# churchill-lab/alntools

Hardware: AMD Instinct MI355X
Metric: alignments/sec BAM->EC (100M PE reads, 8-hap) at 1/2/4/8 MI355X (higher is better)
Workload: dtype u32

## Files before the change

alntools_amd/csrc/ecb.hip:

```cpp
#include <hip/hip_runtime.h>

#include <algorithm>
#include <climits>
#include <cstddef>
#include <cstdarg>
#include <cstdio>
#include <cstring>
#include <cstdlib>
#include <memory>
#include <mutex>
#include <string>
#include <vector>

#include "../../include/ecb.h"

namespace {

typedef unsigned long long u64;
typedef unsigned int u32;
typedef unsigned short u16;

constexpr int TPB = 256;
constexpr u32 MAX_PROBE = 256;
constexpr u32 PENDING = 0xFFFFFFFFu;
constexpr u32 ARENA_CHUNK = 512;
constexpr u32 QSTRIPES = 64;
constexpr u32 ARENA_REGIONS = 64;
constexpr u32 MAX_LOCI = (1u << 26) - 2u;
constexpr u32 MAX_LOCI_SHORT = (1u << 25) - 2u;
constexpr u32 INL = 5;
constexpr u32 DEAD_KEY = 0xFFFFFFFFu;
constexpr u32 SPIN_MAX = 1u << 16;

constexpr u32 ERR_CONTRACT = 1u;
// ... 1549 lines not shown
    const int* ptr = cscptr + (u64)h * (n_loci + 1);
    const u64 j = g - hap_start[h];
    u32 lo = 0, hi = n_loci;
    while (lo < hi) { const u32 m = (lo + hi + 1) >> 1; if ((u64)ptr[m] <= j) lo = m; else hi = m - 1; }
    keys[g] = (u64)(u32)cscidx[g] * n_loci + lo;
    vals[g] = 1u << h;
}
__global__ void k_cv_back_emit(const u64* keys, const u32* vals, const u32* flag, const u32* pos, u64 total, u32 n_loci,
                               int* indices, int* data) {
    const u64 i = blockIdx.x * (u64)blockDim.x + threadIdx.x;
    if (i >= total || !flag[i]) return;
    u32 m = 0;
    for (u64 j = i; j < total && keys[j] == keys[i]; ++j) m |= vals[j];
    indices[pos[i]] = (int)(keys[i] % n_loci);
    data[pos[i]] = (int)m;
}
__global__ void k_cv_back_rowptr(const u64* keys, const u32* pos, u64 total, u32 nnz, u32 n_ecs, u32 n_loci, int* indptr) {
    const u64 e = blockIdx.x * (u64)blockDim.x + threadIdx.x;
    if (e > n_ecs) return;
    const u64 at = lower_bound_u64(keys, total, (u64)e * n_loci);
    indptr[e] = at < total ? (int)pos[at] : (int)nnz;
}

constexpr int CVB = 1024;
__global__ __launch_bounds__(TPB) void k_cv_bits(const int* data, u64 nnz, u64* total) {
    u64 v = 0;
    for (u64 i = blockIdx.x * (u64)TPB + threadIdx.x; i < nnz; i += (u64)gridDim.x * TPB) v += __popc((u32)data[i]);
#pragma unroll
    for (int d = 32; d > 0; d >>= 1) v += __shfl_xor(v, d);
    if ((threadIdx.x & 63u) == 0 && v) atomicAdd(total, v);
}
__global__ void k_cv_keys(const int* indptr, u32 n_ecs, const int* indices, const int* data, u64 nnz, u32 n_loci, u32 n_haps,
                          u64* keys, u32* vals, u32* err) {
    const u64 e = blockIdx.x * (u64)blockDim.x + threadIdx.x;
    if (e >= n_ecs) return;
    const long long a = indptr[e], b = indptr[e + 1];
    if (a < 0 || b < a || (u64)b > nnz || (e == 0 && a != 0)) { atomicOr(err, 1u); return; }
    bool bad = false;
    for (long long i = a; i < b; ++i) {
        const u32 lc = (u32)indices[i], m = (u32)data[i];
        bad |= lc >= n_loci || m == 0u || (m >> n_haps) != 0u;
        keys[i] = ((u64)lc << 32) | (u32)e;
        vals[i] = m;
    }
    if (bad) atomicOr(err, 2u);
}
__global__ __launch_bounds__(TPB) void k_cv_cnt(const u32* masks, u64 nnz, u32 n_haps, u32 nb, u32* blk) {
    __shared__ u32 cnt[32];
    if (threadIdx.x < 32) cnt[threadIdx.x] = 0;
    __syncthreads();
    const u64 i0 = (u64)blockIdx.x * CVB;
#pragma unroll
    for (int r = 0; r < CVB / TPB; ++r) {
        const u64 i = i0 + (u64)r * TPB + threadIdx.x;
        const u32 m = i < nnz ? masks[i] : 0u;
        for (u32 h = 0; h < n_haps; ++h) {
            const u64 bm = __ballot((m >> h) & 1u);
            if ((threadIdx.x & 63u) == 0 && bm) atomicAdd(&cnt[h], (u32)__popcll(bm));
        }
    }
    __syncthreads();
    if (threadIdx.x < n_haps) blk[(u64)threadIdx.x * nb + blockIdx.x] = cnt[threadIdx.x];
}
template <bool VAL>
__global__ __launch_bounds__(TPB) void k_cv_emit(const u64* keys, const u32* masks, u64 nnz, u32 n_haps, u32 n_loci, u32 nb,
                                                 const u32* scan, int* cscidx, u32* headval, const u32* base, const double* values,
                                                 double* cscdata) {
    __shared__ u32 run[32], wcnt[TPB / 64][32];
    const u32 tid = threadIdx.x, lane = tid & 63u, w = tid >> 6;
    if (tid < 32) run[tid] = tid < n_haps ? scan[(u64)tid * nb + blockIdx.x] : 0u;
    const u64 lt = (1ull << lane) - 1ull;
    const u64 i0 = (u64)blockIdx.x * CVB;
    for (int r = 0; r < CVB / TPB; ++r) {
        const u64 i = i0 + (u64)r * TPB + tid;
        const bool have = i < nnz;
        const u64 key = have ? keys[i] : 0ull;
        const u32 m = have ? masks[i] : 0u;
        const u32 lc = (u32)(key >> 32);
        const bool head = have && (i == 0 || (u32)(keys[i - 1] >> 32) != lc);
        for (u32 h = 0; h < n_haps; ++h) {
            const u64 bm = __ballot((m >> h) & 1u);
            if (lane == 0) wcnt[w][h] = (u32)__popcll(bm);
        }
        __syncthreads();
        for (u32 h = 0; h < n_haps; ++h) {
            const u64 bm = __ballot((m >> h) & 1u);
            u32 at = run[h] + (u32)__popcll(bm & lt);
            for (u32 k = 0; k < w; ++k) at += wcnt[k][h];
            if ((m >> h) & 1u) {
                cscidx[at] = (int)(u32)key;
                if (VAL) cscdata[at] = values[base[i] + (u32)__popc(m & ((1u << h) - 1u))];
            }
            if (head) headval[(u64)h * n_loci + lc] = at - scan[(u64)h * nb];
        }
        __syncthreads();
        if (tid < n_haps) { u32 c = 0; for (u32 k = 0; k < TPB / 64; ++k) c += wcnt[k][tid]; run[tid] += c; }
        __syncthreads();
    }
}
__global__ void k_cv_ptr(const u64* keys, u64 nnz, u32 n_loci, u32 n_haps, u32 nb, const u32* scan, const u64* grand, const u32* headval, int* cscptr) {
    const u64 t = blockIdx.x * (u64)blockDim.x + threadIdx.x;
    if (t > n_loci) return;
    const u64 at = lower_bound_u64(keys, nnz, t << 32);
    const u32 t2 = at < nnz ? (u32)(keys[at] >> 32) : 0u;
    for (u32 h = 0; h < n_haps; ++h) {
        const u32 tot = (h + 1 < n_haps ? scan[(u64)(h + 1) * nb] : (u32)*grand) - scan[(u64)h * nb];
        cscptr[(u64)h * (n_loci + 1) + t] = (int)(at < nnz ? headval[(u64)h * n_loci + t2] : tot);
    }
}

__global__ __launch_bounds__(TPB) void k_cvv_bits(const int* data, u64 nnz, u32* bits) {
    const u64 i = blockIdx.x * (u64)TPB + threadIdx.x;
    if (i < nnz) bits[i] = (u32)__popc((u32)data[i]);
}
__global__ __launch_bounds__(TPB) void k_cvv_gather(const u32* idx, const int* data, const u32* bits_excl, u64 nnz, u32* masks, u32* base) {
    const u64 p = blockIdx.x * (u64)TPB + threadIdx.x;
    if (p >= nnz) return;
    const u32 i = idx[p];
    masks[p] = (u32)data[i];
    base[p] = bits_excl[i];
}

__global__ void k_iota(u32* out, u64 n) {
    const u64 i = blockIdx.x * (u64)blockDim.x + threadIdx.x;
    if (i < n) out[i] = (u32)i;
}
__global__ void k_read_ec(const u32* read_slot, u64 n, const u32* rank_of_slot, int* out) {
    const u64 i = blockIdx.x * (u64)blockDim.x + threadIdx.x;
    if (i < n) out[i] = read_slot[i] == 0xFFFFFFFFu ? -1 : (int)rank_of_slot[read_slot[i]];
// ... 15 lines not shown
    const u64 s = A.start[blockIdx.y], n = A.len[blockIdx.y];
    for (u64 i = blockIdx.x * (u64)blockDim.x + threadIdx.x; i < n; i += (u64)gridDim.x * blockDim.x) arena[s + i] = make_uint2(0u, 0u);
}
__global__ void k_clear_slots(Slot* table, const u32* list, u64 n) {
    const u64 i = blockIdx.x * (u64)blockDim.x + threadIdx.x;
    if (i >= n) return;
    uint4* s = reinterpret_cast<uint4*>(table + list[i]);
    const uint4 z = make_uint4(0, 0, 0, 0);
    s[0] = z; s[1] = z; s[2] = z; s[3] = z;
}

#ifndef ECB_RS_TPB
#define ECB_RS_TPB 1024
#endif
constexpr int RS_TPB = ECB_RS_TPB, RS_TILE = 4096, RS_ITEMS = RS_TILE / RS_TPB;
static_assert(RS_TPB >= 256 && RS_TPB % 64 == 0 && RS_TILE % RS_TPB == 0, "one thread per digit among the first 256");
constexpr int RS_MAX_PASSES = 8;
constexpr u32 RS_AGG = 1u << 30, RS_PFX = 2u << 30, RS_VAL = (1u << 30) - 1u;
constexpr u32 RS_SPIN_MAX = 1u << 24;
#ifndef ECB_RS_LOOK
#define ECB_RS_LOOK 4
#endif
constexpr int RS_LOOK = ECB_RS_LOOK;
struct RsShifts { u32 s[RS_MAX_PASSES]; u32 n; };
__global__ __launch_bounds__(RS_TPB) void k_rs_hist_all(const u64* keys, u64 n, RsShifts sh, u32* ghist) {
    __shared__ u32 h[RS_MAX_PASSES][256];
    for (u32 q = threadIdx.x; q < RS_MAX_PASSES * 256; q += RS_TPB) (&h[0][0])[q] = 0;
    __syncthreads();
    for (u64 i = blockIdx.x * (u64)RS_TPB + threadIdx.x; i < n; i += (u64)gridDim.x * RS_TPB) {
        const u64 k = keys[i];
        for (u32 p = 0; p < sh.n; ++p) atomicAdd(&h[p][(u32)(k >> sh.s[p]) & 255u], 1u);
    }
    __syncthreads();
    if (threadIdx.x < 256u) for (u32 p = 0; p < sh.n; ++p) { const u32 c = h[p][threadIdx.x]; if (c) atomicAdd(&ghist[p * 256 + threadIdx.x], c); }
}
__global__ __launch_bounds__(256) void k_rs_bases(const u32* ghist, u32 n_passes, u32* base) {
    __shared__ u32 s_w[4];
    for (u32 p = 0; p < n_passes; ++p) {
        const u32 v = ghist[p * 256 + threadIdx.x];
        const u32 incl = wave_incl_scan(v);
        if ((threadIdx.x & 63u) == 63u) s_w[threadIdx.x >> 6] = incl;
        __syncthreads();
        u32 before = 0;
        for (u32 k = 0; k < (threadIdx.x >> 6); ++k) before += s_w[k];
        base[p * 256 + threadIdx.x] = before + incl - v;
        __syncthreads();
    }
}
__global__ __launch_bounds__(RS_TPB) void k_rs_pass(const u64* kin, const u32* vin, u64 n, u32 shift, const u32* base, u32* desc,
                                                    u32* ticket, u32* err, u64* kout, u32* vout) {
    __shared__ u32 cnt[RS_TPB / 64][256];
    __shared__ u32 dstart[256];
    __shared__ u32 gbase[256];
    __shared__ u32 s_wsum[RS_TPB / 64];
    __shared__ u32 s_tile;
    __shared__ u64 skey[RS_TILE];
    __shared__ u32 sval[RS_TILE];
    const u32 tid = threadIdx.x, lane = tid & 63u, w = tid >> 6;
    if (tid == 0) s_tile = atomicAdd(ticket, 1u);
    for (u32 q = tid; q < (RS_TPB / 64) * 256; q += RS_TPB) (&cnt[0][0])[q] = 0;
    __syncthreads();
    const u32 tile = s_tile;
    const u64 t0 = (u64)tile * RS_TILE;
    if (t0 >= n) return;
    const u64 w0 = t0 + (u64)w * (RS_TILE / (RS_TPB / 64));
    const u64 lt = (1ull << lane) - 1ull;
    u64 key[RS_ITEMS];
    u32 val[RS_ITEMS], rk[RS_ITEMS];
#pragma unroll
    for (int r = 0; r < RS_ITEMS; ++r) {
        const u64 i = w0 + (u64)r * 64 + lane;
        const bool have = i < n;
        key[r] = have ? kin[i] : 0ull;
        val[r] = have ? vin[i] : 0u;
        const u32 d = (u32)(key[r] >> shift) & 255u;
        u64 peers = __ballot(have);
#pragma unroll
        for (int b = 0; b < 8; ++b) {
            const u64 m = __ballot((d >> b) & 1u);
            peers &= ((d >> b) & 1u) ? m : ~m;
        }
        const u32 below = (u32)__popcll(peers & lt);
        u32 bs = 0;
        if (have && below == 0u) bs = atomicAdd(&cnt[w][d], (u32)__popcll(peers));
        bs = __shfl(bs, have ? __ffsll((long long)peers) - 1 : (int)lane);
        rk[r] = bs + below;
    }
    __syncthreads();
    u32 tot = 0;
    const bool dig = tid < 256u;
    const u32 dt = dig ? tid : 0u;
    if (dig) {
#pragma unroll
        for (int k = 0; k < RS_TPB / 64; ++k) { const u32 c = cnt[k][tid]; cnt[k][tid] = tot; tot += c; }
    }
    u32* const mine = desc + (u64)tile * 256 + dt;
    u32 excl = 0;
    if (!dig) {
    } else if (tile == 0) {
        __hip_atomic_store(mine, RS_PFX | tot, __ATOMIC_RELAXED, __HIP_MEMORY_SCOPE_AGENT);
    } else {
        __hip_atomic_store(mine, RS_AGG | tot, __ATOMIC_RELAXED, __HIP_MEMORY_SCOPE_AGENT);
        u32 spins = 0;
        bool done = false;
        for (long long t = (long long)tile - 1; t >= 0 && !done;) {
            u32 v[RS_LOOK];
#pragma unroll
            for (int k = 0; k < RS_LOOK; ++k)
                v[k] = t - k >= 0 ? __hip_atomic_load(desc + (u64)(t - k) * 256 + dt, __ATOMIC_RELAXED, __HIP_MEMORY_SCOPE_AGENT) : 0u;
            int used = 0;
#pragma unroll
            for (int k = 0; k < RS_LOOK; ++k) {
                if (done || used != k || t - k < 0) continue;
                if (v[k] < RS_AGG) continue;
                excl += v[k] & RS_VAL;
                used = k + 1;
                if (v[k] >= RS_PFX) done = true;
            }
            t -= used;
            if (!used) {
                if (++spins > RS_SPIN_MAX) { atomicOr(err, 1u); break; }
                __builtin_amdgcn_s_sleep(1);
            }
        }
        __hip_atomic_store(mine, RS_PFX | ((excl + tot) & RS_VAL), __ATOMIC_RELAXED, __HIP_MEMORY_SCOPE_AGENT);
    }
    if (dig) gbase[tid] = base[tid] + excl;
    {
        const u32 incl = wave_incl_scan(tot);
        if (lane == 63) s_wsum[w] = incl;
        __syncthreads();
        u32 before = 0;
        for (u32 k = 0; k < w; ++k) before += s_wsum[k];
        if (dig) dstart[tid] = before + incl - tot;
    }
    __syncthreads();
#pragma unroll
    for (int r = 0; r < RS_ITEMS; ++r) {
        const u64 i = w0 + (u64)r * 64 + lane;
        if (i < n) {
            const u32 d = (u32)(key[r] >> shift) & 255u;
            const u32 lp = dstart[d] + cnt[w][d] + rk[r];
            skey[lp] = key[r]; sval[lp] = val[r];
        }
    }
    __syncthreads();
    const u32 n_tile = (u32)min((u64)RS_TILE, n - t0);
    for (u32 i = tid; i < n_tile; i += RS_TPB) {
        const u64 k = skey[i];
        const u32 d = (u32)(k >> shift) & 255u;
        const u64 pos = (u64)gbase[d] + (i - dstart[d]);
        if (pos < n) { kout[pos] = k; vout[pos] = sval[i]; }
    }
}
__global__ __launch_bounds__(TPB) void k_or_reduce(const u64* keys, u64 n, u64* out) {
    u64 v = 0;
    for (u64 i = blockIdx.x * (u64)TPB + threadIdx.x; i < n; i += (u64)gridDim.x * TPB) v |= keys[i];
#pragma unroll
    for (int d = 32; d > 0; d >>= 1) v |= __shfl_xor(v, d);
    if ((threadIdx.x & 63u) == 0 && v) atomicOr(out, v);
}
constexpr u32 MSF_LDS_CELLS = 8192;
constexpr int TPB_MSF = 1024;
__global__ __launch_bounds__(TPB_MSF) void k_msf2_cells(const u32* meta, const u32* cnt, u64 n, u32 n_cells, u64* total, u32* firstfile, u32* err) {
    extern __shared__ u32 sh32[];
    const bool lds = n_cells <= MSF_LDS_CELLS;
    u32 *lfile = sh32, *lcnt = sh32 + (lds ? n_cells : 0);
    if (lds) {
        for (u32 c = threadIdx.x; c < n_cells; c += TPB_MSF) { lfile[c] = 0xFFFFFFFFu; lcnt[c] = 0; }
        __syncthreads();
    }
    const u64 per = (n + gridDim.x - 1) / gridDim.x, t0 = blockIdx.x * per, t1 = min(t0 + per, n);
    for (u64 t = t0 + threadIdx.x; t < t1; t += TPB_MSF) {
// ... 721 lines not shown
    HIPCHK(h, scan_launch(h->stream, in, n, out, sums, d_total, stride, last32));
    return ECB_OK;
}
int excl_scan(ecb_handle* h, const u32* in, u64 n, u32* out, u64* total) {
    u64* d_tot = nullptr;
    POOL(h, P_TOTALS, d_tot, 8);
    RCCHK(excl_scan_dev(h, in, n, out, d_tot + 7));
    HIPCHK(h, hipMemcpyAsync(total, d_tot + 7, sizeof(u64), hipMemcpyDeviceToHost, h->stream));
    HIPCHK(h, hipStreamSynchronize(h->stream));
    return ECB_OK;
}

struct SortBufs {
    u64* k[2];
    u32* v[2];
    int at = 0;
    u64* keys() const { return k[at]; }
    u32* vals() const { return v[at]; }
    u64* spare_keys() const { return k[at ^ 1]; }
    u32* spare_vals() const { return v[at ^ 1]; }
};
struct SortScratch { u32 *hist, *offs; u64* d_word; };
inline u64 rs_tiles(u64 n) { return std::max<u64>(1, (n + RS_TILE - 1) / RS_TILE); }
constexpr u64 RS_AUX_WORDS = 2 * RS_MAX_PASSES * 256 + 64;
inline u64 rs_words(u64 n) { return std::max<u64>(256 * rs_tiles(n), RS_AUX_WORDS); }
hipError_t radix_sort_pairs64(hipStream_t st, SortBufs& b, u64 n, const SortScratch& sc, u64 bit_mask = ~0ull) {
    b.at = 0;
    if (n < 2) return hipSuccess;
    if (n >= (1ull << 30)) return hipErrorInvalidValue;
    hipError_t e = hipSuccess;
    u64 ormask = bit_mask;
    if (bit_mask == ~0ull) {
        if ((e = hipMemsetAsync(sc.d_word, 0, 8, st)) != hipSuccess) return e;
        k_or_reduce<<<(unsigned)std::min<u64>(1024, (n + TPB - 1) / TPB), TPB, 0, st>>>(b.k[0], n, sc.d_word);
        if ((e = hipMemcpyAsync(&ormask, sc.d_word, 8, hipMemcpyDeviceToHost, st)) != hipSuccess) return e;
        if ((e = hipStreamSynchronize(st)) != hipSuccess) return e;
    }
    RsShifts sh{};
    for (u32 shift = 0; shift < 64; shift += 8)
        if ((ormask >> shift) & 255ull) sh.s[sh.n++] = shift;
    if (!sh.n) return hipSuccess;
    const u32 nt = (u32)rs_tiles(n);
    u32 *ghist = sc.offs, *base = sc.offs + RS_MAX_PASSES * 256, *ticket = sc.offs + 2 * RS_MAX_PASSES * 256, *err = ticket + 1;
    if ((e = hipMemsetAsync(sc.offs, 0, RS_AUX_WORDS * 4, st)) != hipSuccess) return e;
    k_rs_hist_all<<<(unsigned)std::min<u64>(2048, (n + 16 * RS_TPB - 1) / (16 * RS_TPB)), RS_TPB, 0, st>>>(b.k[0], n, sh, ghist);
    k_rs_bases<<<1, 256, 0, st>>>(ghist, sh.n, base);
    for (u32 p = 0; p < sh.n; ++p) {
        if ((e = hipMemsetAsync(sc.hist, 0, (u64)nt * 256 * 4, st)) != hipSuccess) return e;
        if ((e = hipMemsetAsync(ticket, 0, 4, st)) != hipSuccess) return e;
        k_rs_pass<<<nt, RS_TPB, 0, st>>>(b.keys(), b.vals(), n, sh.s[p], base + p * 256, sc.hist, ticket, err, b.spare_keys(), b.spare_vals());
        b.at ^= 1;
    }
    if ((e = hipGetLastError()) != hipSuccess) return e;
    u32 gave_up = 0;
    if ((e = hipMemcpyAsync(&gave_up, err, 4, hipMemcpyDeviceToHost, st)) != hipSuccess) return e;
    if ((e = hipStreamSynchronize(st)) != hipSuccess) return e;
    return gave_up ? hipErrorUnknown : hipSuccess;
}
int handle_sort(ecb_handle* h, SortBufs& b, u64 n, u64 bit_mask = ~0ull) {
    SortScratch sc{};
    u64* tot = nullptr;
    POOL(h, P_RS_HIST, sc.hist, rs_words(n)); POOL(h, P_RS_OFFS, sc.offs, RS_AUX_WORDS); POOL(h, P_TOTALS, tot, 8);
    sc.d_word = tot + 6;
    HIPCHK_AS(h, "radix sort: ", radix_sort_pairs64(h->stream, b, n, sc, bit_mask));
    return ECB_OK;
}
int sorted_runs(ecb_handle* h, SortBufs& b, u64 n, u32* flag, u32* pos, u64* n_runs) {
    RCCHK(handle_sort(h, b, n));
    k_run_heads<<<nblk(n, TPB), TPB, 0, h->stream>>>(b.keys(), n, flag);
    return excl_scan(h, flag, n, pos, n_runs);
}

int ensure_slot_ranks(ecb_handle* h, u64 E) {
    if (h->run.csr.rank_of_slot) return ECB_OK;
    POOL(h, P_RANK, h->run.csr.rank_of_slot, h->cap);
    k_slot_ranks<<<nblk(E, TPB), TPB, 0, h->stream>>>(h->run.csr.order, E, h->run.csr.rank_of_slot);
    HIPCHK(h, hipGetLastError());
    return ECB_OK;
}

// ... 1162 lines not shown
    hipStream_t st = c.st;
    int nnz_i = 0;
    CALLCHK(c, hipMemcpy(&nnz_i, (const int*)d_indptr + n_ecs, 4, hipMemcpyDeviceToHost));
    if (nnz_i < 0) return fail(nullptr, ECB_ERR_CONTRACT, "malformed CSR: negative row pointer");
    const u64 nnz = (u64)nnz_i;
    if (nnz && (!d_indices || !d_data)) return fail(nullptr, ECB_ERR_ARG, "bad argument");
    u64* words = c.get<u64>(CV_WORDS, 4);
    if (const int rc = c.missing()) return rc;
    if (!d_cscidx || !d_cscptr || (payload && !d_cscdata)) {
        u64 tot = 0;
        CALLCHK(c, hipMemsetAsync(words, 0, 8, st));
        if (nnz) k_cv_bits<<<(unsigned)std::min<u64>(2048, nblk(nnz, TPB)), TPB, 0, st>>>((const int*)d_data, nnz, words);
        if (const int rc = c.read_back(&tot, words, 1)) return rc;
        if (tot >= (1ull << 32)) return fail(nullptr, ECB_ERR_LIMIT, "more than 2^32-1 set haplotype bits");
        *total = tot;
        return ECB_OK;
    }
    const u64 nc = (u64)n_haps * (n_loci + 1);
    if (!nnz) {
        CALLCHK(c, hipMemset(d_cscptr, 0, nc * 4));
        *total = 0;
        return ECB_OK;
    }
    const u32 nb = (u32)nblk(nnz, CVB);
    u64 *k0 = c.get<u64>(CV_KEYS0, nnz), *k1 = c.get<u64>(CV_KEYS1, nnz);
    u32 *v0 = c.get<u32>(CV_VALS0, nnz), *v1 = c.get<u32>(CV_VALS1, nnz);
    SortScratch ss{c.get<u32>(CV_HIST, rs_words(nnz)), c.get<u32>(CV_OFFS, RS_AUX_WORDS), words + 3};
    u32 *blk = c.get<u32>(CV_BLK, (u64)n_haps * nb), *scan = c.get<u32>(CV_SCAN, (u64)n_haps * nb);
    u32 *sums2 = c.get<u32>(CV_SUMS2, scan_words(std::max<u64>((u64)n_haps * nb, payload ? nnz + 1 : 0)) + 2);
    u32* headval = c.get<u32>(CV_HEAD, (u64)n_haps * n_loci);
    u32 *bits = nullptr, *bits_excl = nullptr, *base = nullptr;
    if (payload) { bits = c.get<u32>(CV_X0, nnz); bits_excl = c.get<u32>(CV_X1, nnz + 1); base = c.get<u32>(CV_X2, nnz); }
    if (const int rc = c.missing()) return rc;
    CALLCHK(c, hipMemsetAsync(words, 0, 24, st));
    k_cv_keys<<<nblk(n_ecs, TPB), TPB, 0, st>>>((const int*)d_indptr, n_ecs, (const int*)d_indices, (const int*)d_data, nnz, n_loci, n_haps,
                                               k0, v0, reinterpret_cast<u32*>(words + 2));
    if (payload) {
        k_iota<<<nblk(nnz, TPB), TPB, 0, st>>>(v0, nnz);
        k_cvv_bits<<<nblk(nnz, TPB), TPB, 0, st>>>((const int*)d_data, nnz, bits);
        CALLCHK(c, scan_launch(st, bits, nnz, bits_excl, sums2, nullptr, 1, bits_excl + nnz));
    }
    SortBufs s{{k0, k1}, {v0, v1}};
    CALLCHK(c, radix_sort_pairs64(st, s, nnz, ss, msb_mask(n_loci - 1) << 32));
    const u64* keys = s.keys(); const u32* masks = s.vals();
    if (payload) {
        u32* m2 = s.vals() == v0 ? v1 : v0;
        k_cvv_gather<<<nblk(nnz, TPB), TPB, 0, st>>>(s.vals(), (const int*)d_data, bits_excl, nnz, m2, base);
        masks = m2;
    }
    k_cv_cnt<<<nb, TPB, 0, st>>>(masks, nnz, n_haps, nb, blk);
    CALLCHK(c, scan_launch(st, blk, (u64)n_haps * nb, scan, sums2, words + 1));
    u64 back[3] = {0, 0, 0};
    if (const int rc = c.read_back(back, words, 3)) return rc;
    if (const int rc = refuse_bits(nullptr, CV_ERRS, (u32)back[2])) return rc;
    if (back[1] >= (1ull << 32)) return fail(nullptr, ECB_ERR_LIMIT, "more than 2^32-1 set haplotype bits");
    *total = back[1];
    if (payload && back[1] && !d_values) return fail(nullptr, ECB_ERR_ARG, "bad argument");
    if (payload)
        k_cv_emit<true><<<nb, TPB, 0, st>>>(keys, masks, nnz, n_haps, n_loci, nb, scan, (int*)d_cscidx, headval, base, (const double*)d_values,
                                            (double*)d_cscdata);
    else k_cv_emit<false><<<nb, TPB, 0, st>>>(keys, masks, nnz, n_haps, n_loci, nb, scan, (int*)d_cscidx, headval, nullptr, nullptr, nullptr);
    k_cv_ptr<<<nblk((u64)n_loci + 1, TPB), TPB, 0, st>>>(keys, nnz, n_loci, n_haps, nb, scan, words + 1, headval, (int*)d_cscptr);
    CALLCHK(c, hipStreamSynchronize(st));
    return ECB_OK;
}
}

extern "C" int ecb_csr_to_hapcsc_device(int device, uint32_t n_ecs, uint32_t n_loci, uint32_t n_haps, const void* d_indptr,
                                        const void* d_indices, const void* d_data, void* d_cscptr, void* d_cscidx,
                                        uint64_t* total) {
    return csr_to_hapcsc_any(device, n_ecs, n_loci, n_haps, d_indptr, d_indices, d_data, nullptr, d_cscptr, d_cscidx, nullptr, false, total);
}

extern "C" int ecb_csr_to_hapcsc_values_device(int device, uint32_t n_ecs, uint32_t n_loci, uint32_t n_haps, const void* d_indptr,
                                               const void* d_indices, const void* d_data, const void* d_values, void* d_cscptr,
                                               void* d_cscidx, void* d_cscdata, uint64_t* total) {
    return csr_to_hapcsc_any(device, n_ecs, n_loci, n_haps, d_indptr, d_indices, d_data, d_values, d_cscptr, d_cscidx, d_cscdata, true, total);
}

extern "C" int ecb_hapcsc_to_csr_device(int device, uint32_t n_ecs, uint32_t n_loci, uint32_t n_haps, const void* d_cscptr,
                                        const void* d_cscidx, uint64_t total, void* d_indptr, void* d_indices, void* d_data,
                                        uint64_t* nnz_out) {
    if (!d_cscptr || !d_cscidx || !d_indptr || !d_indices || !d_data || !nnz_out || !n_ecs || !n_loci || !n_haps || n_haps > 31 || !total)
        return fail(nullptr, ECB_ERR_ARG, "bad argument");
    if (total >= (1ull << 32)) return fail(nullptr, ECB_ERR_LIMIT, "more than 2^32-1 row indices");
    Call c(device, ""); if (c.rc) return c.rc;
// ... 1819 lines not shown
```

alntools_amd/csrc/quant.inc:

```
namespace {
constexpr u32 Q_LONG_ROW = 256;
constexpr u32 Q_LONG_COL = 32;
constexpr u32 Q_TILE = 2048;
constexpr u32 Q_BATCH = 8;
enum : u32 { Q_ERR_SCALE = 1u, Q_ERR_THETA = 2u, Q_ERR_GENE = 4u };
struct QState {
    u32 done, n_iter, converged, max_iters;
    double delta, stop;
    u64 explained, W;
    u32 n_long_rows, n_long_cols;
};
const ErrBit Q_ERRS[] = {
    {Q_ERR_SCALE, ECB_ERR_CONTRACT, "ecquant: an entry of scale is NaN, infinite or negative"},
    {Q_ERR_THETA, ECB_ERR_CONTRACT, "ecquant: an entry of theta_in is NaN, infinite or negative"},
    {Q_ERR_GENE, ECB_ERR_CONTRACT, "ecquant: a gene id outside [0, n_genes)"},
};
template <class V> __device__ __forceinline__ V q_block_sum(V v, V* s, u32 stop = 1) {
    s[threadIdx.x] = v;
    __syncthreads();
    for (u32 k = TPB / 2; k >= stop; k >>= 1) {
        if (threadIdx.x < k) s[threadIdx.x] += s[threadIdx.x + k];
        __syncthreads();
    }
    return s[threadIdx.x < stop ? threadIdx.x : 0];
// ... 237 lines not shown
    CALLCHK(c, hipMemsetAsync(f.words, 0, n_words * 8, st));
    if (m.pn) {
        CALLCHK(c, hipMemsetAsync(f.ww, 0, std::max<u64>(m.n_ecs, 1) * 8, st));
        k_ca_weights<<<nblk(std::max<u64>(m.nnz_n, (u64)m.n_samples + 1), TPB), TPB, 0, st>>>(m.pn, m.n_samples, m.xn, m.dn, m.nnz_n, m.n_ecs, sample, f.ww,
                                                                                             f.words);
    }
    k_gm_check<true><<<nblk(std::max<u64>((u64)m.n_ecs + 1, (nnz + GM_ITEMS - 1) / GM_ITEMS), TPB), TPB, 0, st>>>(m.ip, m.n_ecs, m.ix, m.da, nnz, nullptr,
                                                                                                               m.n_loci, m.n_haps, bits, f.words);
    CALLCHK(c, hipGetLastError());
    CALLCHK(c, scan_launch(st, bits, nnz, f.bits_excl, f.sums, f.words + 3, 1, f.bits_excl + nnz));
    if (d_scale) k_q_tab<<<nblk(n_tab, TPB), TPB, 0, st>>>((const double*)d_scale, m.n_loci, m.n_haps, f.scale, Q_ERR_SCALE, err);
    if (d_theta) k_q_tab<<<nblk(n_tab, TPB), TPB, 0, st>>>((const double*)d_theta, m.n_loci, m.n_haps, f.theta, theta_bit, err);
    if (gene && m.n_loci) k_qm_gkeys<<<nblk(m.n_loci, TPB), TPB, 0, st>>>(gene, m.n_loci, n_genes, f.gk[0], f.gv[0], err);
    CALLCHK(c, hipGetLastError());
    f.back.resize(n_words);
    if (const int rc = c.read_back(f.back.data(), f.words, n_words, GM_ERRS)) return rc;
    RCCHK(ca_refuse_input(f.back));
    if (f.back[3] >= (1ull << 32)) return fail(nullptr, ECB_ERR_LIMIT, "more than 2^32-1 set haplotype bits");
    RCCHK(refuse_bits(nullptr, errs, (u32)f.back[5]));
    f.n_bits = f.back[3];
    return ECB_OK;
}

struct QSort { SortBufs s; SortScratch ss; };
QSort q_sort_bufs(Call& c, u64 n, u64 n_hist, u64* d_word) {
    u64 *k0 = c.get<u64>(CV_KEYS0, n), *k1 = c.get<u64>(CV_KEYS1, n);
    u32 *v0 = c.get<u32>(CV_VALS0, n), *v1 = c.get<u32>(CV_VALS1, n);
    return QSort{SortBufs{{k0, k1}, {v0, v1}}, SortScratch{c.get<u32>(CV_HIST, rs_words(n_hist)), c.get<u32>(CV_OFFS, RS_AUX_WORDS), d_word}};
}

struct QCols { int *colptr, *col_ec, *col_mask; u32* col_b0; };
__global__ __launch_bounds__(TPB) void k_qm_colbase(const u64* ckeys, u64 nnz, const int* indptr, const int* indices, const u32* bits_excl, u32* col_b0);
int q_col_view(Call& c, const QMat& m, const QFront& f, QSort& srt, bool with_b0, QCols& v) {
    hipStream_t st = c.st;
    const u64 nnz = m.nnz;
    v = QCols{c.get<int>((u64)m.n_loci + 1), c.get<int>(nnz), c.get<int>(nnz), with_b0 ? c.get<u32>(nnz) : nullptr};
    if (const int rc = c.missing()) return rc;
    k_cv_keys<<<nblk(m.n_ecs, TPB), TPB, 0, st>>>(m.ip, m.n_ecs, m.ix, m.da, nnz, m.n_loci, m.n_haps, srt.s.k[0], srt.s.v[0],
                                                 reinterpret_cast<u32*>(f.words + 6));
    CALLCHK(c, radix_sort_pairs64(st, srt.s, nnz, srt.ss, msb_mask(m.n_loci - 1) << 32));
    k_split_out<<<nblk(nnz, TPB), TPB, 0, st>>>(srt.s.keys(), srt.s.vals(), nnz, v.col_ec, v.col_mask);
    k_row_ptr<<<nblk((u64)m.n_loci + 1, TPB), TPB, 0, st>>>(srt.s.keys(), nnz, m.n_loci, v.colptr);
    if (with_b0) k_qm_colbase<<<nblk(nnz, TPB), TPB, 0, st>>>(srt.s.keys(), nnz, m.ip, m.ix, f.bits_excl, v.col_b0);
    CALLCHK(c, hipGetLastError());
    return ECB_OK;
}

struct QView {
    hipStream_t st;
    u32 n_ecs, n_loci, n_haps, hp, n_eblk, n_parts, nlr, nlc; u64 nnz;
    const int *ip, *ix, *da;
    const u32 *bits_excl, *long_rows, *long_cols;
    QCols cols;
    const u64* ww;
    const QState* qs;
    const double* scale;
    double *theta, *phi, *acc_long, *partial;
    u64* expl_parts;
};
struct QGenes {
    u32 n_genes;
    int *gptr, *gmem; u32* long_genes;
    const u64* rkeys; const u32* gnz;
// ... 144 lines not shown
```

Baseline: 361.3 billion.

## Use wider radix digits, per-wave chunk counts, and defer readback in column conversion

The radix sort is templated on digit width. Column conversion and quant use 9-bit digits with 16-bit packed shared counters, so fewer passes are needed for the loci key range. The count and emit kernels move from 1024-element block tiles with shared memory and barriers to one wave per 64-element chunk, using shuffles instead of __syncthreads. The host sync and readback in between are removed: emit and ptr launch right away and check device-side refusal flags, so errors are read once at the end. The cost is a larger per-chunk scan and wasted kernel work on refused inputs.

```diff
diff --git a/alntools_amd/csrc/ecb.hip b/alntools_amd/csrc/ecb.hip
--- a/alntools_amd/csrc/ecb.hip
+++ b/alntools_amd/csrc/ecb.hip
@@ -10,6 +10,7 @@
 #include <memory>
 #include <mutex>
 #include <string>
+#include <type_traits>
 #include <vector>
 
 #include "../../include/ecb.h"
@@ -1605,7 +1606,6 @@
     indptr[e] = at < total ? (int)pos[at] : (int)nnz;
 }
 
-constexpr int CVB = 1024;
 __global__ __launch_bounds__(TPB) void k_cv_bits(const int* data, u64 nnz, u64* total) {
     u64 v = 0;
     for (u64 i = blockIdx.x * (u64)TPB + threadIdx.x; i < nnz; i += (u64)gridDim.x * TPB) v += __popc((u32)data[i]);
@@ -1628,66 +1628,59 @@
     }
     if (bad) atomicOr(err, 2u);
 }
-__global__ __launch_bounds__(TPB) void k_cv_cnt(const u32* masks, u64 nnz, u32 n_haps, u32 nb, u32* blk) {
-    __shared__ u32 cnt[32];
-    if (threadIdx.x < 32) cnt[threadIdx.x] = 0;
-    __syncthreads();
-    const u64 i0 = (u64)blockIdx.x * CVB;
-#pragma unroll
-    for (int r = 0; r < CVB / TPB; ++r) {
-        const u64 i = i0 + (u64)r * TPB + threadIdx.x;
-        const u32 m = i < nnz ? masks[i] : 0u;
-        for (u32 h = 0; h < n_haps; ++h) {
-            const u64 bm = __ballot((m >> h) & 1u);
-            if ((threadIdx.x & 63u) == 0 && bm) atomicAdd(&cnt[h], (u32)__popcll(bm));
-        }
-    }
-    __syncthreads();
-    if (threadIdx.x < n_haps) blk[(u64)threadIdx.x * nb + blockIdx.x] = cnt[threadIdx.x];
+__device__ __forceinline__ bool cv_refused(const u64* words) { return (words[2] | words[3] | (words[1] >> 32)) != 0ull; }
+__global__ __launch_bounds__(TPB) void k_cv_cnt(const u32* masks, u64 nnz, u32 n_haps, u32 nc, u32* cnt) {
+    const u64 c = blockIdx.x * (u64)(TPB / 64) + (threadIdx.x >> 6);
+    if (c >= nc) return;
+    const u32 lane = threadIdx.x & 63u;
+    const u64 i = c * 64 + lane;
+    const u32 m = i < nnz ? masks[i] : 0u;
+    u32 mine = 0;
+    for (u32 h = 0; h < n_haps; ++h) {
+        const u32 k = (u32)__popcll(__ballot((m >> h) & 1u));
+        if (lane == h) mine = k;
+    }
+    if (lane < n_haps) cnt[(u64)lane * nc + c] = mine;
 }
 template <bool VAL>
-__global__ __launch_bounds__(TPB) void k_cv_emit(const u64* keys, const u32* masks, u64 nnz, u32 n_haps, u32 n_loci, u32 nb,
-                                                 const u32* scan, int* cscidx, u32* headval, const u32* base, const double* values,
-                                                 double* cscdata) {
-    __shared__ u32 run[32], wcnt[TPB / 64][32];
-    const u32 tid = threadIdx.x, lane = tid & 63u, w = tid >> 6;
-    if (tid < 32) run[tid] = tid < n_haps ? scan[(u64)tid * nb + blockIdx.x] : 0u;
+__global__ __launch_bounds__(TPB) void k_cv_emit(const u64* keys, const u32* masks, u64 nnz, u32 n_haps, u32 n_loci, u32 nc,
+                                                 const u32* scan, const u64* words, int* cscidx, u32* headval,
+                                                 const u32* base, const double* values, double* cscdata) {
+    const u64 c = blockIdx.x * (u64)(TPB / 64) + (threadIdx.x >> 6);
+    if (c >= nc || cv_refused(words)) return;
+    const u32 lane = threadIdx.x & 63u;
     const u64 lt = (1ull << lane) - 1ull;
-    const u64 i0 = (u64)blockIdx.x * CVB;
-    for (int r = 0; r < CVB / TPB; ++r) {
-        const u64 i = i0 + (u64)r * TPB + tid;
-        const bool have = i < nnz;
-        const u64 key = have ? keys[i] : 0ull;
-        const u32 m = have ? masks[i] : 0u;
-        const u32 lc = (u32)(key >> 32);
-        const bool head = have && (i == 0 || (u32)(keys[i - 1] >> 32) != lc);
-        for (u32 h = 0; h < n_haps; ++h) {
-            const u64 bm = __ballot((m >> h) & 1u);
-            if (lane == 0) wcnt[w][h] = (u32)__popcll(bm);
-        }
-        __syncthreads();
-        for (u32 h = 0; h < n_haps; ++h) {
-            const u64 bm = __ballot((m >> h) & 1u);
-            u32 at = run[h] + (u32)__popcll(bm & lt);
-            for (u32 k = 0; k < w; ++k) at += wcnt[k][h];
-            if ((m >> h) & 1u) {
-                cscidx[at] = (int)(u32)key;
-                if (VAL) cscdata[at] = values[base[i] + (u32)__popc(m & ((1u << h) - 1u))];
-            }
-            if (head) headval[(u64)h * n_loci + lc] = at - scan[(u64)h * nb];
-        }
-        __syncthreads();
-        if (tid < n_haps) { u32 c = 0; for (u32 k = 0; k < TPB / 64; ++k) c += wcnt[k][tid]; run[tid] += c; }
-        __syncthreads();
-    }
-}
-__global__ void k_cv_ptr(const u64* keys, u64 nnz, u32 n_loci, u32 n_haps, u32 nb, const u32* scan, const u64* grand, const u32* headval, int* cscptr) {
+    const u64 i = c * 64 + lane;
+    const bool have = i < nnz;
+    const u64 key = have ? keys[i] : 0ull;
+    const u32 m = have ? masks[i] : 0u;
+    const u32 lc = (u32)(key >> 32);
+    u32 prev = __shfl_up(lc, 1);
+    if (lane == 0 && i > 0) prev = (u32)(keys[i - 1] >> 32);
+    const bool head = have && (i == 0 || prev != lc);
+    u32 first = 0, hap0 = 0;
+    if (lane < n_haps) { first = scan[(u64)lane * nc + c]; hap0 = scan[(u64)lane * nc]; }
+    u32 vb = 0;
+    if (VAL) vb = have ? base[i] : 0u;
+    for (u32 h = 0; h < n_haps; ++h) {
+        const u64 bm = __ballot((m >> h) & 1u);
+        const u32 at = (u32)__shfl((int)first, (int)h) + (u32)__popcll(bm & lt);
+        const u32 h0 = (u32)__shfl((int)hap0, (int)h);
+        if ((m >> h) & 1u) {
+            cscidx[at] = (int)(u32)key;
+            if (VAL) cscdata[at] = values[vb + (u32)__popc(m & ((1u << h) - 1u))];
+        }
+        if (head) headval[(u64)h * n_loci + lc] = at - h0;
+    }
+}
+__global__ void k_cv_ptr(const u64* keys, u64 nnz, u32 n_loci, u32 n_haps, u32 nc, const u32* scan, const u64* words, const u32* headval,
+                         int* cscptr) {
     const u64 t = blockIdx.x * (u64)blockDim.x + threadIdx.x;
-    if (t > n_loci) return;
+    if (t > n_loci || cv_refused(words)) return;
     const u64 at = lower_bound_u64(keys, nnz, t << 32);
     const u32 t2 = at < nnz ? (u32)(keys[at] >> 32) : 0u;
     for (u32 h = 0; h < n_haps; ++h) {
-        const u32 tot = (h + 1 < n_haps ? scan[(u64)(h + 1) * nb] : (u32)*grand) - scan[(u64)h * nb];
+        const u32 tot = (h + 1 < n_haps ? scan[(u64)(h + 1) * nc] : (u32)words[1]) - scan[(u64)h * nc];
         cscptr[(u64)h * (n_loci + 1) + t] = (int)(at < nnz ? headval[(u64)h * n_loci + t2] : tot);
     }
 }
@@ -1749,43 +1742,61 @@
 #define ECB_RS_LOOK 4
 #endif
 constexpr int RS_LOOK = ECB_RS_LOOK;
-struct RsShifts { u32 s[RS_MAX_PASSES]; u32 n; };
+struct RsShifts { u32 s[RS_MAX_PASSES], m[RS_MAX_PASSES]; u32 n; };
+typedef u32 __attribute__((may_alias)) u32_alias;
+template <int BITS> struct RsDigit {
+    static_assert(BITS >= 8 && (1 << BITS) <= RS_TPB, "one thread per digit");
+    static constexpr u32 D = 1u << BITS;
+    using cnt_t = std::conditional_t<BITS == 8, u32, unsigned short>;
+};
+__device__ __forceinline__ u32 rs_bump(u32* row, u32 d, u32 by) { return atomicAdd(&row[d], by); }
+__device__ __forceinline__ u32 rs_bump(unsigned short* row, u32 d, u32 by) {
+    const u32 sh = (d & 1u) * 16u;
+    return (atomicAdd(reinterpret_cast<u32_alias*>(row) + (d >> 1), by << sh) >> sh) & 0xFFFFu;
+}
+template <int BITS>
 __global__ __launch_bounds__(RS_TPB) void k_rs_hist_all(const u64* keys, u64 n, RsShifts sh, u32* ghist) {
-    __shared__ u32 h[RS_MAX_PASSES][256];
-    for (u32 q = threadIdx.x; q < RS_MAX_PASSES * 256; q += RS_TPB) (&h[0][0])[q] = 0;
+    constexpr u32 D = RsDigit<BITS>::D;
+    __shared__ u32 h[RS_MAX_PASSES][D];
+    for (u32 q = threadIdx.x; q < RS_MAX_PASSES * D; q += RS_TPB) (&h[0][0])[q] = 0;
     __syncthreads();
     for (u64 i = blockIdx.x * (u64)RS_TPB + threadIdx.x; i < n; i += (u64)gridDim.x * RS_TPB) {
         const u64 k = keys[i];
-        for (u32 p = 0; p < sh.n; ++p) atomicAdd(&h[p][(u32)(k >> sh.s[p]) & 255u], 1u);
+        for (u32 p = 0; p < sh.n; ++p) atomicAdd(&h[p][(u32)(k >> sh.s[p]) & sh.m[p]], 1u);
     }
     __syncthreads();
-    if (threadIdx.x < 256u) for (u32 p = 0; p < sh.n; ++p) { const u32 c = h[p][threadIdx.x]; if (c) atomicAdd(&ghist[p * 256 + threadIdx.x], c); }
-}
-__global__ __launch_bounds__(256) void k_rs_bases(const u32* ghist, u32 n_passes, u32* base) {
-    __shared__ u32 s_w[4];
+    if (threadIdx.x < D) for (u32 p = 0; p < sh.n; ++p) { const u32 c = h[p][threadIdx.x]; if (c) atomicAdd(&ghist[p * D + threadIdx.x], c); }
+}
+template <int BITS>
+__global__ __launch_bounds__(1 << BITS) void k_rs_bases(const u32* ghist, u32 n_passes, u32* base) {
+    constexpr u32 D = RsDigit<BITS>::D;
+    __shared__ u32 s_w[D / 64];
     for (u32 p = 0; p < n_passes; ++p) {
-        const u32 v = ghist[p * 256 + threadIdx.x];
+        const u32 v = ghist[p * D + threadIdx.x];
         const u32 incl = wave_incl_scan(v);
         if ((threadIdx.x & 63u) == 63u) s_w[threadIdx.x >> 6] = incl;
         __syncthreads();
         u32 before = 0;
         for (u32 k = 0; k < (threadIdx.x >> 6); ++k) before += s_w[k];
-        base[p * 256 + threadIdx.x] = before + incl - v;
+        base[p * D + threadIdx.x] = before + incl - v;
         __syncthreads();
     }
 }
-__global__ __launch_bounds__(RS_TPB) void k_rs_pass(const u64* kin, const u32* vin, u64 n, u32 shift, const u32* base, u32* desc,
+template <int BITS>
+__global__ __launch_bounds__(RS_TPB) void k_rs_pass(const u64* kin, const u32* vin, u64 n, u32 shift, u32 dmask, const u32* base, u32* desc,
                                                     u32* ticket, u32* err, u64* kout, u32* vout) {
-    __shared__ u32 cnt[RS_TPB / 64][256];
-    __shared__ u32 dstart[256];
-    __shared__ u32 gbase[256];
+    constexpr u32 D = RsDigit<BITS>::D;
+    using cnt_t = typename RsDigit<BITS>::cnt_t;
+    __shared__ __attribute__((aligned(4))) cnt_t cnt[RS_TPB / 64][D];
+    __shared__ u32 dstart[D];
+    __shared__ u32 gbase[D];
     __shared__ u32 s_wsum[RS_TPB / 64];
     __shared__ u32 s_tile;
     __shared__ u64 skey[RS_TILE];
     __shared__ u32 sval[RS_TILE];
     const u32 tid = threadIdx.x, lane = tid & 63u, w = tid >> 6;
     if (tid == 0) s_tile = atomicAdd(ticket, 1u);
-    for (u32 q = tid; q < (RS_TPB / 64) * 256; q += RS_TPB) (&cnt[0][0])[q] = 0;
+    for (u32 q = tid; q < (RS_TPB / 64) * D; q += RS_TPB) (&cnt[0][0])[q] = 0;
     __syncthreads();
     const u32 tile = s_tile;
     const u64 t0 = (u64)tile * RS_TILE;
@@ -1800,28 +1811,28 @@
         const bool have = i < n;
         key[r] = have ? kin[i] : 0ull;
         val[r] = have ? vin[i] : 0u;
-        const u32 d = (u32)(key[r] >> shift) & 255u;
+        const u32 d = (u32)(key[r] >> shift) & dmask;
         u64 peers = __ballot(have);
 #pragma unroll
-        for (int b = 0; b < 8; ++b) {
+        for (int b = 0; b < BITS; ++b) {
             const u64 m = __ballot((d >> b) & 1u);
             peers &= ((d >> b) & 1u) ? m : ~m;
         }
         const u32 below = (u32)__popcll(peers & lt);
         u32 bs = 0;
-        if (have && below == 0u) bs = atomicAdd(&cnt[w][d], (u32)__popcll(peers));
+        if (have && below == 0u) bs = rs_bump(cnt[w], d, (u32)__popcll(peers));
         bs = __shfl(bs, have ? __ffsll((long long)peers) - 1 : (int)lane);
         rk[r] = bs + below;
     }
     __syncthreads();
     u32 tot = 0;
-    const bool dig = tid < 256u;
+    const bool dig = tid < D;
     const u32 dt = dig ? tid : 0u;
     if (dig) {
 #pragma unroll
-        for (int k = 0; k < RS_TPB / 64; ++k) { const u32 c = cnt[k][tid]; cnt[k][tid] = tot; tot += c; }
-    }
-    u32* const mine = desc + (u64)tile * 256 + dt;
+        for (int k = 0; k < RS_TPB / 64; ++k) { const u32 c = cnt[k][tid]; cnt[k][tid] = (cnt_t)tot; tot += c; }
+    }
+    u32* const mine = desc + (u64)tile * D + dt;
     u32 excl = 0;
     if (!dig) {
     } else if (tile == 0) {
@@ -1834,7 +1845,7 @@
             u32 v[RS_LOOK];
 #pragma unroll
             for (int k = 0; k < RS_LOOK; ++k)
-                v[k] = t - k >= 0 ? __hip_atomic_load(desc + (u64)(t - k) * 256 + dt, __ATOMIC_RELAXED, __HIP_MEMORY_SCOPE_AGENT) : 0u;
+                v[k] = t - k >= 0 ? __hip_atomic_load(desc + (u64)(t - k) * D + dt, __ATOMIC_RELAXED, __HIP_MEMORY_SCOPE_AGENT) : 0u;
             int used = 0;
 #pragma unroll
             for (int k = 0; k < RS_LOOK; ++k) {
@@ -1866,7 +1877,7 @@
     for (int r = 0; r < RS_ITEMS; ++r) {
         const u64 i = w0 + (u64)r * 64 + lane;
         if (i < n) {
-            const u32 d = (u32)(key[r] >> shift) & 255u;
+            const u32 d = (u32)(key[r] >> shift) & dmask;
             const u32 lp = dstart[d] + cnt[w][d] + rk[r];
             skey[lp] = key[r]; sval[lp] = val[r];
         }
@@ -1875,7 +1886,7 @@
     const u32 n_tile = (u32)min((u64)RS_TILE, n - t0);
     for (u32 i = tid; i < n_tile; i += RS_TPB) {
         const u64 k = skey[i];
-        const u32 d = (u32)(k >> shift) & 255u;
+        const u32 d = (u32)(k >> shift) & dmask;
         const u64 pos = (u64)gbase[d] + (i - dstart[d]);
         if (pos < n) { kout[pos] = k; vout[pos] = sval[i]; }
     }
@@ -2643,13 +2654,32 @@
 };
 struct SortScratch { u32 *hist, *offs; u64* d_word; };
 inline u64 rs_tiles(u64 n) { return std::max<u64>(1, (n + RS_TILE - 1) / RS_TILE); }
-constexpr u64 RS_AUX_WORDS = 2 * RS_MAX_PASSES * 256 + 64;
-inline u64 rs_words(u64 n) { return std::max<u64>(256 * rs_tiles(n), RS_AUX_WORDS); }
-hipError_t radix_sort_pairs64(hipStream_t st, SortBufs& b, u64 n, const SortScratch& sc, u64 bit_mask = ~0ull) {
+template <int BITS> constexpr u64 rs_aux_words() { return 2ull * RS_MAX_PASSES * (1u << BITS) + 64; }
+constexpr u64 RS_AUX_WORDS = rs_aux_words<8>();
+template <int BITS = 8> inline u64 rs_words(u64 n) { return std::max<u64>(((u64)1 << BITS) * rs_tiles(n), rs_aux_words<BITS>()); }
+template <int BITS> RsShifts rs_plan(u64 ormask) {
+    RsShifts sh{};
+    if (BITS == 8) {
+        for (u32 shift = 0; shift < 64; shift += 8)
+            if ((ormask >> shift) & 255ull) { sh.m[sh.n] = 255u; sh.s[sh.n++] = shift; }
+    } else if (ormask) {
+        u32 shift = (u32)__builtin_ctzll(ormask), left = 64u - (u32)__builtin_clzll(ormask) - shift;
+        for (u32 np = (left + BITS - 1) / BITS; np; --np) {
+            const u32 wd = (left + np - 1) / np;
+            sh.m[sh.n] = (1u << wd) - 1u; sh.s[sh.n++] = shift;
+            shift += wd; left -= wd;
+        }
+    }
+    return sh;
+}
+template <int BITS = 8>
+hipError_t radix_sort_pairs64(hipStream_t st, SortBufs& b, u64 n, const SortScratch& sc, u64 bit_mask = ~0ull, u32* gave_up = nullptr) {
+    constexpr u32 D = 1u << BITS;
     b.at = 0;
+    u32 *ghist = sc.offs, *base = sc.offs + RS_MAX_PASSES * D, *ticket = sc.offs + 2 * RS_MAX_PASSES * D, *err = gave_up ? gave_up : ticket + 1;
+    hipError_t e = hipSuccess;
     if (n < 2) return hipSuccess;
     if (n >= (1ull << 30)) return hipErrorInvalidValue;
-    hipError_t e = hipSuccess;
     u64 ormask = bit_mask;
     if (bit_mask == ~0ull) {
         if ((e = hipMemsetAsync(sc.d_word, 0, 8, st)) != hipSuccess) return e;
@@ -2657,26 +2687,25 @@
         if ((e = hipMemcpyAsync(&ormask, sc.d_word, 8, hipMemcpyDeviceToHost, st)) != hipSuccess) return e;
         if ((e = hipStreamSynchronize(st)) != hipSuccess) return e;
     }
-    RsShifts sh{};
-    for (u32 shift = 0; shift < 64; shift += 8)
-        if ((ormask >> shift) & 255ull) sh.s[sh.n++] = shift;
+    const RsShifts sh = rs_plan<BITS>(ormask);
     if (!sh.n) return hipSuccess;
     const u32 nt = (u32)rs_tiles(n);
-    u32 *ghist = sc.offs, *base = sc.offs + RS_MAX_PASSES * 256, *ticket = sc.offs + 2 * RS_MAX_PASSES * 256, *err = ticket + 1;
-    if ((e = hipMemsetAsync(sc.offs, 0, RS_AUX_WORDS * 4, st)) != hipSuccess) return e;
-    k_rs_hist_all<<<(unsigned)std::min<u64>(2048, (n + 16 * RS_TPB - 1) / (16 * RS_TPB)), RS_TPB, 0, st>>>(b.k[0], n, sh, ghist);
-    k_rs_bases<<<1, 256, 0, st>>>(ghist, sh.n, base);
+    if ((e = hipMemsetAsync(sc.offs, 0, rs_aux_words<BITS>() * 4, st)) != hipSuccess) return e;
+    k_rs_hist_all<BITS><<<(unsigned)std::min<u64>(2048, (n + 16 * RS_TPB - 1) / (16 * RS_TPB)), RS_TPB, 0, st>>>(b.k[0], n, sh, ghist);
+    k_rs_bases<BITS><<<1, D, 0, st>>>(ghist, sh.n, base);
     for (u32 p = 0; p < sh.n; ++p) {
-        if ((e = hipMemsetAsync(sc.hist, 0, (u64)nt * 256 * 4, st)) != hipSuccess) return e;
+        if ((e = hipMemsetAsync(sc.hist, 0, (u64)nt * D * 4, st)) != hipSuccess) return e;
         if ((e = hipMemsetAsync(ticket, 0, 4, st)) != hipSuccess) return e;
-        k_rs_pass<<<nt, RS_TPB, 0, st>>>(b.keys(), b.vals(), n, sh.s[p], base + p * 256, sc.hist, ticket, err, b.spare_keys(), b.spare_vals());
+        k_rs_pass<BITS><<<nt, RS_TPB, 0, st>>>(b.keys(), b.vals(), n, sh.s[p], sh.m[p], base + p * D, sc.hist, ticket, err, b.spare_keys(),
+                                               b.spare_vals());
         b.at ^= 1;
     }
     if ((e = hipGetLastError()) != hipSuccess) return e;
-    u32 gave_up = 0;
-    if ((e = hipMemcpyAsync(&gave_up, err, 4, hipMemcpyDeviceToHost, st)) != hipSuccess) return e;
+    if (gave_up) return hipSuccess;
+    u32 bad = 0;
+    if ((e = hipMemcpyAsync(&bad, err, 4, hipMemcpyDeviceToHost, st)) != hipSuccess) return e;
     if ((e = hipStreamSynchronize(st)) != hipSuccess) return e;
-    return gave_up ? hipErrorUnknown : hipSuccess;
+    return bad ? hipErrorUnknown : hipSuccess;
 }
 int handle_sort(ecb_handle* h, SortBufs& b, u64 n, u64 bit_mask = ~0ull) {
     SortScratch sc{};
@@ -3885,17 +3914,18 @@
         *total = 0;
         return ECB_OK;
     }
-    const u32 nb = (u32)nblk(nnz, CVB);
+    constexpr int CV_BITS = 9;
+    const u32 nch = (u32)nblk(nnz, 64);
     u64 *k0 = c.get<u64>(CV_KEYS0, nnz), *k1 = c.get<u64>(CV_KEYS1, nnz);
     u32 *v0 = c.get<u32>(CV_VALS0, nnz), *v1 = c.get<u32>(CV_VALS1, nnz);
-    SortScratch ss{c.get<u32>(CV_HIST, rs_words(nnz)), c.get<u32>(CV_OFFS, RS_AUX_WORDS), words + 3};
-    u32 *blk = c.get<u32>(CV_BLK, (u64)n_haps * nb), *scan = c.get<u32>(CV_SCAN, (u64)n_haps * nb);
-    u32 *sums2 = c.get<u32>(CV_SUMS2, scan_words(std::max<u64>((u64)n_haps * nb, payload ? nnz + 1 : 0)) + 2);
+    SortScratch ss{c.get<u32>(CV_HIST, rs_words<CV_BITS>(nnz)), c.get<u32>(CV_OFFS, rs_aux_words<CV_BITS>()), nullptr};
+    u32 *cnt = c.get<u32>(CV_BLK, (u64)n_haps * nch), *scan = c.get<u32>(CV_SCAN, (u64)n_haps * nch);
+    u32 *sums2 = c.get<u32>(CV_SUMS2, scan_words(std::max<u64>((u64)n_haps * nch, payload ? nnz + 1 : 0)) + 2);
     u32* headval = c.get<u32>(CV_HEAD, (u64)n_haps * n_loci);
     u32 *bits = nullptr, *bits_excl = nullptr, *base = nullptr;
     if (payload) { bits = c.get<u32>(CV_X0, nnz); bits_excl = c.get<u32>(CV_X1, nnz + 1); base = c.get<u32>(CV_X2, nnz); }
     if (const int rc = c.missing()) return rc;
-    CALLCHK(c, hipMemsetAsync(words, 0, 24, st));
+    CALLCHK(c, hipMemsetAsync(words, 0, 32, st));
     k_cv_keys<<<nblk(n_ecs, TPB), TPB, 0, st>>>((const int*)d_indptr, n_ecs, (const int*)d_indices, (const int*)d_data, nnz, n_loci, n_haps,
                                                k0, v0, reinterpret_cast<u32*>(words + 2));
     if (payload) {
@@ -3904,27 +3934,32 @@
         CALLCHK(c, scan_launch(st, bits, nnz, bits_excl, sums2, nullptr, 1, bits_excl + nnz));
     }
     SortBufs s{{k0, k1}, {v0, v1}};
-    CALLCHK(c, radix_sort_pairs64(st, s, nnz, ss, msb_mask(n_loci - 1) << 32));
+    CALLCHK(c, radix_sort_pairs64<CV_BITS>(st, s, nnz, ss, msb_mask(n_loci - 1) << 32, reinterpret_cast<u32*>(words + 3)));
     const u64* keys = s.keys(); const u32* masks = s.vals();
     if (payload) {
         u32* m2 = s.vals() == v0 ? v1 : v0;
         k_cvv_gather<<<nblk(nnz, TPB), TPB, 0, st>>>(s.vals(), (const int*)d_data, bits_excl, nnz, m2, base);
         masks = m2;
     }
-    k_cv_cnt<<<nb, TPB, 0, st>>>(masks, nnz, n_haps, nb, blk);
-    CALLCHK(c, scan_launch(st, blk, (u64)n_haps * nb, scan, sums2, words + 1));
-    u64 back[3] = {0, 0, 0};
-    if (const int rc = c.read_back(back, words, 3)) return rc;
+    const unsigned grid = (unsigned)nblk(nch, TPB / 64);
+    k_cv_cnt<<<grid, TPB, 0, st>>>(masks, nnz, n_haps, nch, cnt);
+    CALLCHK(c, scan_launch(st, cnt, (u64)n_haps * nch, scan, sums2, words + 1));
+    if (payload && d_values)
+        k_cv_emit<true><<<grid, TPB, 0, st>>>(keys, masks, nnz, n_haps, n_loci, nch, scan, words, (int*)d_cscidx, headval, base,
+                                              (const double*)d_values, (double*)d_cscdata);
+    else if (!payload)
+        k_cv_emit<false><<<grid, TPB, 0, st>>>(keys, masks, nnz, n_haps, n_loci, nch, scan, words, (int*)d_cscidx, headval, nullptr, nullptr,
+                                               nullptr);
+    if (!payload || d_values)
+        k_cv_ptr<<<nblk((u64)n_loci + 1, TPB), TPB, 0, st>>>(keys, nnz, n_loci, n_haps, nch, scan, words, headval, (int*)d_cscptr);
+    CALLCHK(c, hipGetLastError());
+    u64 back[4] = {0, 0, 0, 0};
+    if (const int rc = c.read_back(back, words, 4)) return rc;
+    if (back[3]) CALLCHK(c, hipErrorUnknown);
     if (const int rc = refuse_bits(nullptr, CV_ERRS, (u32)back[2])) return rc;
     if (back[1] >= (1ull << 32)) return fail(nullptr, ECB_ERR_LIMIT, "more than 2^32-1 set haplotype bits");
     *total = back[1];
     if (payload && back[1] && !d_values) return fail(nullptr, ECB_ERR_ARG, "bad argument");
-    if (payload)
-        k_cv_emit<true><<<nb, TPB, 0, st>>>(keys, masks, nnz, n_haps, n_loci, nb, scan, (int*)d_cscidx, headval, base, (const double*)d_values,
-                                            (double*)d_cscdata);
-    else k_cv_emit<false><<<nb, TPB, 0, st>>>(keys, masks, nnz, n_haps, n_loci, nb, scan, (int*)d_cscidx, headval, nullptr, nullptr, nullptr);
-    k_cv_ptr<<<nblk((u64)n_loci + 1, TPB), TPB, 0, st>>>(keys, nnz, n_loci, n_haps, nb, scan, words + 1, headval, (int*)d_cscptr);
-    CALLCHK(c, hipStreamSynchronize(st));
     return ECB_OK;
 }
 }
diff --git a/alntools_amd/csrc/quant.inc b/alntools_amd/csrc/quant.inc
--- a/alntools_amd/csrc/quant.inc
+++ b/alntools_amd/csrc/quant.inc
@@ -283,11 +283,12 @@
     return ECB_OK;
 }
 
+constexpr int Q_COL_BITS = 9;
 struct QSort { SortBufs s; SortScratch ss; };
 QSort q_sort_bufs(Call& c, u64 n, u64 n_hist, u64* d_word) {
     u64 *k0 = c.get<u64>(CV_KEYS0, n), *k1 = c.get<u64>(CV_KEYS1, n);
     u32 *v0 = c.get<u32>(CV_VALS0, n), *v1 = c.get<u32>(CV_VALS1, n);
-    return QSort{SortBufs{{k0, k1}, {v0, v1}}, SortScratch{c.get<u32>(CV_HIST, rs_words(n_hist)), c.get<u32>(CV_OFFS, RS_AUX_WORDS), d_word}};
+    return QSort{SortBufs{{k0, k1}, {v0, v1}}, SortScratch{c.get<u32>(CV_HIST, rs_words<Q_COL_BITS>(n_hist)), c.get<u32>(CV_OFFS, rs_aux_words<Q_COL_BITS>()), d_word}};
 }
 
 struct QCols { int *colptr, *col_ec, *col_mask; u32* col_b0; };
@@ -299,7 +300,7 @@
     if (const int rc = c.missing()) return rc;
     k_cv_keys<<<nblk(m.n_ecs, TPB), TPB, 0, st>>>(m.ip, m.n_ecs, m.ix, m.da, nnz, m.n_loci, m.n_haps, srt.s.k[0], srt.s.v[0],
                                                  reinterpret_cast<u32*>(f.words + 6));
-    CALLCHK(c, radix_sort_pairs64(st, srt.s, nnz, srt.ss, msb_mask(m.n_loci - 1) << 32));
+    CALLCHK(c, radix_sort_pairs64<Q_COL_BITS>(st, srt.s, nnz, srt.ss, msb_mask(m.n_loci - 1) << 32));
     k_split_out<<<nblk(nnz, TPB), TPB, 0, st>>>(srt.s.keys(), srt.s.vals(), nnz, v.col_ec, v.col_mask);
     k_row_ptr<<<nblk((u64)m.n_loci + 1, TPB), TPB, 0, st>>>(srt.s.keys(), nnz, m.n_loci, v.colptr);
     if (with_b0) k_qm_colbase<<<nblk(nnz, TPB), TPB, 0, st>>>(srt.s.keys(), nnz, m.ip, m.ix, f.bits_excl, v.col_b0);
```

Result: no change. 359.2 billion (median of 2 runs) (-0.6%).
